# google/compare_gan

Measured on NVIDIA H100. Metric: images/sec G+D step (resnet_cifar10), higher is better.
Workload: dtype tf32

## Files before the change

### compare_gan_b200/csrc/wgmma_tf32.cuh

```cuda
#pragma once
#include <stdint.h>

namespace tc {

template <int N>
__device__ __forceinline__ void wgmma_tf32(float* d, uint64_t da, uint64_t db);

template <>
__device__ __forceinline__ void wgmma_tf32<32>(float* d, uint64_t da, uint64_t db) {
  asm volatile(
      "{\n\t.reg .pred p;\n\tsetp.ne.b32 p, %18, 0;\n\t"
      "wgmma.mma_async.sync.aligned.m64n32k8.f32.tf32.tf32 {%0, %1, %2, %3, %4, %5, %6, %7, %8, %9, %10, %11, %12, %13, %14, %15}, %16, %17, p, 1, 1;\n\t}\n"
      : "+f"(d[0]), "+f"(d[1]), "+f"(d[2]), "+f"(d[3]), "+f"(d[4]), "+f"(d[5]), "+f"(d[6]), "+f"(d[7]), "+f"(d[8]), "+f"(d[9]), "+f"(d[10]), "+f"(d[11]), "+f"(d[12]), "+f"(d[13]), "+f"(d[14]), "+f"(d[15])
      : "l"(da), "l"(db), "r"(1));
}

template <>
__device__ __forceinline__ void wgmma_tf32<64>(float* d, uint64_t da, uint64_t db) {
  asm volatile(
      "{\n\t.reg .pred p;\n\tsetp.ne.b32 p, %34, 0;\n\t"
      "wgmma.mma_async.sync.aligned.m64n64k8.f32.tf32.tf32 {%0, %1, %2, %3, %4, %5, %6, %7, %8, %9, %10, %11, %12, %13, %14, %15, %16, %17, %18, %19, %20, %21, %22, %23, %24, %25, %26, %27, %28, %29, %30, %31}, %32, %33, p, 1, 1;\n\t}\n"
      : "+f"(d[0]), "+f"(d[1]), "+f"(d[2]), "+f"(d[3]), "+f"(d[4]), "+f"(d[5]), "+f"(d[6]), "+f"(d[7]), "+f"(d[8]), "+f"(d[9]), "+f"(d[10]), "+f"(d[11]), "+f"(d[12]), "+f"(d[13]), "+f"(d[14]), "+f"(d[15]), "+f"(d[16]), "+f"(d[17]), "+f"(d[18]), "+f"(d[19]), "+f"(d[20]), "+f"(d[21]), "+f"(d[22]), "+f"(d[23]), "+f"(d[24]), "+f"(d[25]), "+f"(d[26]), "+f"(d[27]), "+f"(d[28]), "+f"(d[29]), "+f"(d[30]), "+f"(d[31])
      : "l"(da), "l"(db), "r"(1));
}

template <>
__device__ __forceinline__ void wgmma_tf32<96>(float* d, uint64_t da, uint64_t db) {
  asm volatile(
      "{\n\t.reg .pred p;\n\tsetp.ne.b32 p, %50, 0;\n\t"
      "wgmma.mma_async.sync.aligned.m64n96k8.f32.tf32.tf32 {%0, %1, %2, %3, %4, %5, %6, %7, %8, %9, %10, %11, %12, %13, %14, %15, %16, %17, %18, %19, %20, %21, %22, %23, %24, %25, %26, %27, %28, %29, %30, %31, %32, %33, %34, %35, %36, %37, %38, %39, %40, %41, %42, %43, %44, %45, %46, %47}, %48, %49, p, 1, 1;\n\t}\n"
      : "+f"(d[0]), "+f"(d[1]), "+f"(d[2]), "+f"(d[3]), "+f"(d[4]), "+f"(d[5]), "+f"(d[6]), "+f"(d[7]), "+f"(d[8]), "+f"(d[9]), "+f"(d[10]), "+f"(d[11]), "+f"(d[12]), "+f"(d[13]), "+f"(d[14]), "+f"(d[15]), "+f"(d[16]), "+f"(d[17]), "+f"(d[18]), "+f"(d[19]), "+f"(d[20]), "+f"(d[21]), "+f"(d[22]), "+f"(d[23]), "+f"(d[24]), "+f"(d[25]), "+f"(d[26]), "+f"(d[27]), "+f"(d[28]), "+f"(d[29]), "+f"(d[30]), "+f"(d[31]), "+f"(d[32]), "+f"(d[33]), "+f"(d[34]), "+f"(d[35]), "+f"(d[36]), "+f"(d[37]), "+f"(d[38]), "+f"(d[39]), "+f"(d[40]), "+f"(d[41]), "+f"(d[42]), "+f"(d[43]), "+f"(d[44]), "+f"(d[45]), "+f"(d[46]), "+f"(d[47])
      : "l"(da), "l"(db), "r"(1));
}

template <>
__device__ __forceinline__ void wgmma_tf32<128>(float* d, uint64_t da, uint64_t db) {
  asm volatile(
      "{\n\t.reg .pred p;\n\tsetp.ne.b32 p, %66, 0;\n\t"
      "wgmma.mma_async.sync.aligned.m64n128k8.f32.tf32.tf32 {%0, %1, %2, %3, %4, %5, %6, %7, %8, %9, %10, %11, %12, %13, %14, %15, %16, %17, %18, %19, %20, %21, %22, %23, %24, %25, %26, %27, %28, %29, %30, %31, %32, %33, %34, %35, %36, %37, %38, %39, %40, %41, %42, %43, %44, %45, %46, %47, %48, %49, %50, %51, %52, %53, %54, %55, %56, %57, %58, %59, %60, %61, %62, %63}, %64, %65, p, 1, 1;\n\t}\n"
      : "+f"(d[0]), "+f"(d[1]), "+f"(d[2]), "+f"(d[3]), "+f"(d[4]), "+f"(d[5]), "+f"(d[6]), "+f"(d[7]), "+f"(d[8]), "+f"(d[9]), "+f"(d[10]), "+f"(d[11]), "+f"(d[12]), "+f"(d[13]), "+f"(d[14]), "+f"(d[15]), "+f"(d[16]), "+f"(d[17]), "+f"(d[18]), "+f"(d[19]), "+f"(d[20]), "+f"(d[21]), "+f"(d[22]), "+f"(d[23]), "+f"(d[24]), "+f"(d[25]), "+f"(d[26]), "+f"(d[27]), "+f"(d[28]), "+f"(d[29]), "+f"(d[30]), "+f"(d[31]), "+f"(d[32]), "+f"(d[33]), "+f"(d[34]), "+f"(d[35]), "+f"(d[36]), "+f"(d[37]), "+f"(d[38]), "+f"(d[39]), "+f"(d[40]), "+f"(d[41]), "+f"(d[42]), "+f"(d[43]), "+f"(d[44]), "+f"(d[45]), "+f"(d[46]), "+f"(d[47]), "+f"(d[48]), "+f"(d[49]), "+f"(d[50]), "+f"(d[51]), "+f"(d[52]), "+f"(d[53]), "+f"(d[54]), "+f"(d[55]), "+f"(d[56]), "+f"(d[57]), "+f"(d[58]), "+f"(d[59]), "+f"(d[60]), "+f"(d[61]), "+f"(d[62]), "+f"(d[63])
      : "l"(da), "l"(db), "r"(1));
}

template <>
__device__ __forceinline__ void wgmma_tf32<160>(float* d, uint64_t da, uint64_t db) {
  asm volatile(
      "{\n\t.reg .pred p;\n\tsetp.ne.b32 p, %82, 0;\n\t"
      "wgmma.mma_async.sync.aligned.m64n160k8.f32.tf32.tf32 {%0, %1, %2, %3, %4, %5, %6, %7, %8, %9, %10, %11, %12, %13, %14, %15, %16, %17, %18, %19, %20, %21, %22, %23, %24, %25, %26, %27, %28, %29, %30, %31, %32, %33, %34, %35, %36, %37, %38, %39, %40, %41, %42, %43, %44, %45, %46, %47, %48, %49, %50, %51, %52, %53, %54, %55, %56, %57, %58, %59, %60, %61, %62, %63, %64, %65, %66, %67, %68, %69, %70, %71, %72, %73, %74, %75, %76, %77, %78, %79}, %80, %81, p, 1, 1;\n\t}\n"
      : "+f"(d[0]), "+f"(d[1]), "+f"(d[2]), "+f"(d[3]), "+f"(d[4]), "+f"(d[5]), "+f"(d[6]), "+f"(d[7]), "+f"(d[8]), "+f"(d[9]), "+f"(d[10]), "+f"(d[11]), "+f"(d[12]), "+f"(d[13]), "+f"(d[14]), "+f"(d[15]), "+f"(d[16]), "+f"(d[17]), "+f"(d[18]), "+f"(d[19]), "+f"(d[20]), "+f"(d[21]), "+f"(d[22]), "+f"(d[23]), "+f"(d[24]), "+f"(d[25]), "+f"(d[26]), "+f"(d[27]), "+f"(d[28]), "+f"(d[29]), "+f"(d[30]), "+f"(d[31]), "+f"(d[32]), "+f"(d[33]), "+f"(d[34]), "+f"(d[35]), "+f"(d[36]), "+f"(d[37]), "+f"(d[38]), "+f"(d[39]), "+f"(d[40]), "+f"(d[41]), "+f"(d[42]), "+f"(d[43]), "+f"(d[44]), "+f"(d[45]), "+f"(d[46]), "+f"(d[47]), "+f"(d[48]), "+f"(d[49]), "+f"(d[50]), "+f"(d[51]), "+f"(d[52]), "+f"(d[53]), "+f"(d[54]), "+f"(d[55]), "+f"(d[56]), "+f"(d[57]), "+f"(d[58]), "+f"(d[59]), "+f"(d[60]), "+f"(d[61]), "+f"(d[62]), "+f"(d[63]), "+f"(d[64]), "+f"(d[65]), "+f"(d[66]), "+f"(d[67]), "+f"(d[68]), "+f"(d[69]), "+f"(d[70]), "+f"(d[71]), "+f"(d[72]), "+f"(d[73]), "+f"(d[74]), "+f"(d[75]), "+f"(d[76]), "+f"(d[77]), "+f"(d[78]), "+f"(d[79])
      : "l"(da), "l"(db), "r"(1));
}

template <>
__device__ __forceinline__ void wgmma_tf32<192>(float* d, uint64_t da, uint64_t db) {
  asm volatile(
      "{\n\t.reg .pred p;\n\tsetp.ne.b32 p, %98, 0;\n\t"
      "wgmma.mma_async.sync.aligned.m64n192k8.f32.tf32.tf32 {%0, %1, %2, %3, %4, %5, %6, %7, %8, %9, %10, %11, %12, %13, %14, %15, %16, %17, %18, %19, %20, %21, %22, %23, %24, %25, %26, %27, %28, %29, %30, %31, %32, %33, %34, %35, %36, %37, %38, %39, %40, %41, %42, %43, %44, %45, %46, %47, %48, %49, %50, %51, %52, %53, %54, %55, %56, %57, %58, %59, %60, %61, %62, %63, %64, %65, %66, %67, %68, %69, %70, %71, %72, %73, %74, %75, %76, %77, %78, %79, %80, %81, %82, %83, %84, %85, %86, %87, %88, %89, %90, %91, %92, %93, %94, %95}, %96, %97, p, 1, 1;\n\t}\n"
      : "+f"(d[0]), "+f"(d[1]), "+f"(d[2]), "+f"(d[3]), "+f"(d[4]), "+f"(d[5]), "+f"(d[6]), "+f"(d[7]), "+f"(d[8]), "+f"(d[9]), "+f"(d[10]), "+f"(d[11]), "+f"(d[12]), "+f"(d[13]), "+f"(d[14]), "+f"(d[15]), "+f"(d[16]), "+f"(d[17]), "+f"(d[18]), "+f"(d[19]), "+f"(d[20]), "+f"(d[21]), "+f"(d[22]), "+f"(d[23]), "+f"(d[24]), "+f"(d[25]), "+f"(d[26]), "+f"(d[27]), "+f"(d[28]), "+f"(d[29]), "+f"(d[30]), "+f"(d[31]), "+f"(d[32]), "+f"(d[33]), "+f"(d[34]), "+f"(d[35]), "+f"(d[36]), "+f"(d[37]), "+f"(d[38]), "+f"(d[39]), "+f"(d[40]), "+f"(d[41]), "+f"(d[42]), "+f"(d[43]), "+f"(d[44]), "+f"(d[45]), "+f"(d[46]), "+f"(d[47]), "+f"(d[48]), "+f"(d[49]), "+f"(d[50]), "+f"(d[51]), "+f"(d[52]), "+f"(d[53]), "+f"(d[54]), "+f"(d[55]), "+f"(d[56]), "+f"(d[57]), "+f"(d[58]), "+f"(d[59]), "+f"(d[60]), "+f"(d[61]), "+f"(d[62]), "+f"(d[63]), "+f"(d[64]), "+f"(d[65]), "+f"(d[66]), "+f"(d[67]), "+f"(d[68]), "+f"(d[69]), "+f"(d[70]), "+f"(d[71]), "+f"(d[72]), "+f"(d[73]), "+f"(d[74]), "+f"(d[75]), "+f"(d[76]), "+f"(d[77]), "+f"(d[78]), "+f"(d[79]), "+f"(d[80]), "+f"(d[81]), "+f"(d[82]), "+f"(d[83]), "+f"(d[84]), "+f"(d[85]), "+f"(d[86]), "+f"(d[87]), "+f"(d[88]), "+f"(d[89]), "+f"(d[90]), "+f"(d[91]), "+f"(d[92]), "+f"(d[93]), "+f"(d[94]), "+f"(d[95])
      : "l"(da), "l"(db), "r"(1));
}

template <>
__device__ __forceinline__ void wgmma_tf32<224>(float* d, uint64_t da, uint64_t db) {
  asm volatile(
      "{\n\t.reg .pred p;\n\tsetp.ne.b32 p, %114, 0;\n\t"
      "wgmma.mma_async.sync.aligned.m64n224k8.f32.tf32.tf32 {%0, %1, %2, %3, %4, %5, %6, %7, %8, %9, %10, %11, %12, %13, %14, %15, %16, %17, %18, %19, %20, %21, %22, %23, %24, %25, %26, %27, %28, %29, %30, %31, %32, %33, %34, %35, %36, %37, %38, %39, %40, %41, %42, %43, %44, %45, %46, %47, %48, %49, %50, %51, %52, %53, %54, %55, %56, %57, %58, %59, %60, %61, %62, %63, %64, %65, %66, %67, %68, %69, %70, %71, %72, %73, %74, %75, %76, %77, %78, %79, %80, %81, %82, %83, %84, %85, %86, %87, %88, %89, %90, %91, %92, %93, %94, %95, %96, %97, %98, %99, %100, %101, %102, %103, %104, %105, %106, %107, %108, %109, %110, %111}, %112, %113, p, 1, 1;\n\t}\n"
      : "+f"(d[0]), "+f"(d[1]), "+f"(d[2]), "+f"(d[3]), "+f"(d[4]), "+f"(d[5]), "+f"(d[6]), "+f"(d[7]), "+f"(d[8]), "+f"(d[9]), "+f"(d[10]), "+f"(d[11]), "+f"(d[12]), "+f"(d[13]), "+f"(d[14]), "+f"(d[15]), "+f"(d[16]), "+f"(d[17]), "+f"(d[18]), "+f"(d[19]), "+f"(d[20]), "+f"(d[21]), "+f"(d[22]), "+f"(d[23]), "+f"(d[24]), "+f"(d[25]), "+f"(d[26]), "+f"(d[27]), "+f"(d[28]), "+f"(d[29]), "+f"(d[30]), "+f"(d[31]), "+f"(d[32]), "+f"(d[33]), "+f"(d[34]), "+f"(d[35]), "+f"(d[36]), "+f"(d[37]), "+f"(d[38]), "+f"(d[39]), "+f"(d[40]), "+f"(d[41]), "+f"(d[42]), "+f"(d[43]), "+f"(d[44]), "+f"(d[45]), "+f"(d[46]), "+f"(d[47]), "+f"(d[48]), "+f"(d[49]), "+f"(d[50]), "+f"(d[51]), "+f"(d[52]), "+f"(d[53]), "+f"(d[54]), "+f"(d[55]), "+f"(d[56]), "+f"(d[57]), "+f"(d[58]), "+f"(d[59]), "+f"(d[60]), "+f"(d[61]), "+f"(d[62]), "+f"(d[63]), "+f"(d[64]), "+f"(d[65]), "+f"(d[66]), "+f"(d[67]), "+f"(d[68]), "+f"(d[69]), "+f"(d[70]), "+f"(d[71]), "+f"(d[72]), "+f"(d[73]), "+f"(d[74]), "+f"(d[75]), "+f"(d[76]), "+f"(d[77]), "+f"(d[78]), "+f"(d[79]), "+f"(d[80]), "+f"(d[81]), "+f"(d[82]), "+f"(d[83]), "+f"(d[84]), "+f"(d[85]), "+f"(d[86]), "+f"(d[87]), "+f"(d[88]), "+f"(d[89]), "+f"(d[90]), "+f"(d[91]), "+f"(d[92]), "+f"(d[93]), "+f"(d[94]), "+f"(d[95]), "+f"(d[96]), "+f"(d[97]), "+f"(d[98]), "+f"(d[99]), "+f"(d[100]), "+f"(d[101]), "+f"(d[102]), "+f"(d[103]), "+f"(d[104]), "+f"(d[105]), "+f"(d[106]), "+f"(d[107]), "+f"(d[108]), "+f"(d[109]), "+f"(d[110]), "+f"(d[111])
      : "l"(da), "l"(db), "r"(1));
}

template <>
__device__ __forceinline__ void wgmma_tf32<256>(float* d, uint64_t da, uint64_t db) {
  asm volatile(
      "{\n\t.reg .pred p;\n\tsetp.ne.b32 p, %130, 0;\n\t"
      "wgmma.mma_async.sync.aligned.m64n256k8.f32.tf32.tf32 {%0, %1, %2, %3, %4, %5, %6, %7, %8, %9, %10, %11, %12, %13, %14, %15, %16, %17, %18, %19, %20, %21, %22, %23, %24, %25, %26, %27, %28, %29, %30, %31, %32, %33, %34, %35, %36, %37, %38, %39, %40, %41, %42, %43, %44, %45, %46, %47, %48, %49, %50, %51, %52, %53, %54, %55, %56, %57, %58, %59, %60, %61, %62, %63, %64, %65, %66, %67, %68, %69, %70, %71, %72, %73, %74, %75, %76, %77, %78, %79, %80, %81, %82, %83, %84, %85, %86, %87, %88, %89, %90, %91, %92, %93, %94, %95, %96, %97, %98, %99, %100, %101, %102, %103, %104, %105, %106, %107, %108, %109, %110, %111, %112, %113, %114, %115, %116, %117, %118, %119, %120, %121, %122, %123, %124, %125, %126, %127}, %128, %129, p, 1, 1;\n\t}\n"
      : "+f"(d[0]), "+f"(d[1]), "+f"(d[2]), "+f"(d[3]), "+f"(d[4]), "+f"(d[5]), "+f"(d[6]), "+f"(d[7]), "+f"(d[8]), "+f"(d[9]), "+f"(d[10]), "+f"(d[11]), "+f"(d[12]), "+f"(d[13]), "+f"(d[14]), "+f"(d[15]), "+f"(d[16]), "+f"(d[17]), "+f"(d[18]), "+f"(d[19]), "+f"(d[20]), "+f"(d[21]), "+f"(d[22]), "+f"(d[23]), "+f"(d[24]), "+f"(d[25]), "+f"(d[26]), "+f"(d[27]), "+f"(d[28]), "+f"(d[29]), "+f"(d[30]), "+f"(d[31]), "+f"(d[32]), "+f"(d[33]), "+f"(d[34]), "+f"(d[35]), "+f"(d[36]), "+f"(d[37]), "+f"(d[38]), "+f"(d[39]), "+f"(d[40]), "+f"(d[41]), "+f"(d[42]), "+f"(d[43]), "+f"(d[44]), "+f"(d[45]), "+f"(d[46]), "+f"(d[47]), "+f"(d[48]), "+f"(d[49]), "+f"(d[50]), "+f"(d[51]), "+f"(d[52]), "+f"(d[53]), "+f"(d[54]), "+f"(d[55]), "+f"(d[56]), "+f"(d[57]), "+f"(d[58]), "+f"(d[59]), "+f"(d[60]), "+f"(d[61]), "+f"(d[62]), "+f"(d[63]), "+f"(d[64]), "+f"(d[65]), "+f"(d[66]), "+f"(d[67]), "+f"(d[68]), "+f"(d[69]), "+f"(d[70]), "+f"(d[71]), "+f"(d[72]), "+f"(d[73]), "+f"(d[74]), "+f"(d[75]), "+f"(d[76]), "+f"(d[77]), "+f"(d[78]), "+f"(d[79]), "+f"(d[80]), "+f"(d[81]), "+f"(d[82]), "+f"(d[83]), "+f"(d[84]), "+f"(d[85]), "+f"(d[86]), "+f"(d[87]), "+f"(d[88]), "+f"(d[89]), "+f"(d[90]), "+f"(d[91]), "+f"(d[92]), "+f"(d[93]), "+f"(d[94]), "+f"(d[95]), "+f"(d[96]), "+f"(d[97]), "+f"(d[98]), "+f"(d[99]), "+f"(d[100]), "+f"(d[101]), "+f"(d[102]), "+f"(d[103]), "+f"(d[104]), "+f"(d[105]), "+f"(d[106]), "+f"(d[107]), "+f"(d[108]), "+f"(d[109]), "+f"(d[110]), "+f"(d[111]), "+f"(d[112]), "+f"(d[113]), "+f"(d[114]), "+f"(d[115]), "+f"(d[116]), "+f"(d[117]), "+f"(d[118]), "+f"(d[119]), "+f"(d[120]), "+f"(d[121]), "+f"(d[122]), "+f"(d[123]), "+f"(d[124]), "+f"(d[125]), "+f"(d[126]), "+f"(d[127])
      : "l"(da), "l"(db), "r"(1));
}

template <int N>
__device__ __forceinline__ void wgmma_tf32_rs(float* d, const uint32_t* a, uint64_t db);

template <>
__device__ __forceinline__ void wgmma_tf32_rs<32>(float* d, const uint32_t* a, uint64_t db) {
  asm volatile(
      "{\n\t.reg .pred p;\n\tsetp.ne.b32 p, %21, 0;\n\t"
      "wgmma.mma_async.sync.aligned.m64n32k8.f32.tf32.tf32 {%0, %1, %2, %3, %4, %5, %6, %7, %8, %9, %10, %11, %12, %13, %14, %15}, {%16, %17, %18, %19}, %20, p, 1, 1;\n\t}\n"
      : "+f"(d[0]), "+f"(d[1]), "+f"(d[2]), "+f"(d[3]), "+f"(d[4]), "+f"(d[5]), "+f"(d[6]), "+f"(d[7]), "+f"(d[8]), "+f"(d[9]), "+f"(d[10]), "+f"(d[11]), "+f"(d[12]), "+f"(d[13]), "+f"(d[14]), "+f"(d[15])
      : "r"(a[0]), "r"(a[1]), "r"(a[2]), "r"(a[3]), "l"(db), "r"(1));
}

template <>
__device__ __forceinline__ void wgmma_tf32_rs<64>(float* d, const uint32_t* a, uint64_t db) {
  asm volatile(
      "{\n\t.reg .pred p;\n\tsetp.ne.b32 p, %37, 0;\n\t"
      "wgmma.mma_async.sync.aligned.m64n64k8.f32.tf32.tf32 {%0, %1, %2, %3, %4, %5, %6, %7, %8, %9, %10, %11, %12, %13, %14, %15, %16, %17, %18, %19, %20, %21, %22, %23, %24, %25, %26, %27, %28, %29, %30, %31}, {%32, %33, %34, %35}, %36, p, 1, 1;\n\t}\n"
      : "+f"(d[0]), "+f"(d[1]), "+f"(d[2]), "+f"(d[3]), "+f"(d[4]), "+f"(d[5]), "+f"(d[6]), "+f"(d[7]), "+f"(d[8]), "+f"(d[9]), "+f"(d[10]), "+f"(d[11]), "+f"(d[12]), "+f"(d[13]), "+f"(d[14]), "+f"(d[15]), "+f"(d[16]), "+f"(d[17]), "+f"(d[18]), "+f"(d[19]), "+f"(d[20]), "+f"(d[21]), "+f"(d[22]), "+f"(d[23]), "+f"(d[24]), "+f"(d[25]), "+f"(d[26]), "+f"(d[27]), "+f"(d[28]), "+f"(d[29]), "+f"(d[30]), "+f"(d[31])
      : "r"(a[0]), "r"(a[1]), "r"(a[2]), "r"(a[3]), "l"(db), "r"(1));
}

template <>
__device__ __forceinline__ void wgmma_tf32_rs<96>(float* d, const uint32_t* a, uint64_t db) {
  asm volatile(
      "{\n\t.reg .pred p;\n\tsetp.ne.b32 p, %53, 0;\n\t"
      "wgmma.mma_async.sync.aligned.m64n96k8.f32.tf32.tf32 {%0, %1, %2, %3, %4, %5, %6, %7, %8, %9, %10, %11, %12, %13, %14, %15, %16, %17, %18, %19, %20, %21, %22, %23, %24, %25, %26, %27, %28, %29, %30, %31, %32, %33, %34, %35, %36, %37, %38, %39, %40, %41, %42, %43, %44, %45, %46, %47}, {%48, %49, %50, %51}, %52, p, 1, 1;\n\t}\n"
      : "+f"(d[0]), "+f"(d[1]), "+f"(d[2]), "+f"(d[3]), "+f"(d[4]), "+f"(d[5]), "+f"(d[6]), "+f"(d[7]), "+f"(d[8]), "+f"(d[9]), "+f"(d[10]), "+f"(d[11]), "+f"(d[12]), "+f"(d[13]), "+f"(d[14]), "+f"(d[15]), "+f"(d[16]), "+f"(d[17]), "+f"(d[18]), "+f"(d[19]), "+f"(d[20]), "+f"(d[21]), "+f"(d[22]), "+f"(d[23]), "+f"(d[24]), "+f"(d[25]), "+f"(d[26]), "+f"(d[27]), "+f"(d[28]), "+f"(d[29]), "+f"(d[30]), "+f"(d[31]), "+f"(d[32]), "+f"(d[33]), "+f"(d[34]), "+f"(d[35]), "+f"(d[36]), "+f"(d[37]), "+f"(d[38]), "+f"(d[39]), "+f"(d[40]), "+f"(d[41]), "+f"(d[42]), "+f"(d[43]), "+f"(d[44]), "+f"(d[45]), "+f"(d[46]), "+f"(d[47])
      : "r"(a[0]), "r"(a[1]), "r"(a[2]), "r"(a[3]), "l"(db), "r"(1));
}

template <>
__device__ __forceinline__ void wgmma_tf32_rs<128>(float* d, const uint32_t* a, uint64_t db) {
  asm volatile(
      "{\n\t.reg .pred p;\n\tsetp.ne.b32 p, %69, 0;\n\t"
      "wgmma.mma_async.sync.aligned.m64n128k8.f32.tf32.tf32 {%0, %1, %2, %3, %4, %5, %6, %7, %8, %9, %10, %11, %12, %13, %14, %15, %16, %17, %18, %19, %20, %21, %22, %23, %24, %25, %26, %27, %28, %29, %30, %31, %32, %33, %34, %35, %36, %37, %38, %39, %40, %41, %42, %43, %44, %45, %46, %47, %48, %49, %50, %51, %52, %53, %54, %55, %56, %57, %58, %59, %60, %61, %62, %63}, {%64, %65, %66, %67}, %68, p, 1, 1;\n\t}\n"
      : "+f"(d[0]), "+f"(d[1]), "+f"(d[2]), "+f"(d[3]), "+f"(d[4]), "+f"(d[5]), "+f"(d[6]), "+f"(d[7]), "+f"(d[8]), "+f"(d[9]), "+f"(d[10]), "+f"(d[11]), "+f"(d[12]), "+f"(d[13]), "+f"(d[14]), "+f"(d[15]), "+f"(d[16]), "+f"(d[17]), "+f"(d[18]), "+f"(d[19]), "+f"(d[20]), "+f"(d[21]), "+f"(d[22]), "+f"(d[23]), "+f"(d[24]), "+f"(d[25]), "+f"(d[26]), "+f"(d[27]), "+f"(d[28]), "+f"(d[29]), "+f"(d[30]), "+f"(d[31]), "+f"(d[32]), "+f"(d[33]), "+f"(d[34]), "+f"(d[35]), "+f"(d[36]), "+f"(d[37]), "+f"(d[38]), "+f"(d[39]), "+f"(d[40]), "+f"(d[41]), "+f"(d[42]), "+f"(d[43]), "+f"(d[44]), "+f"(d[45]), "+f"(d[46]), "+f"(d[47]), "+f"(d[48]), "+f"(d[49]), "+f"(d[50]), "+f"(d[51]), "+f"(d[52]), "+f"(d[53]), "+f"(d[54]), "+f"(d[55]), "+f"(d[56]), "+f"(d[57]), "+f"(d[58]), "+f"(d[59]), "+f"(d[60]), "+f"(d[61]), "+f"(d[62]), "+f"(d[63])
      : "r"(a[0]), "r"(a[1]), "r"(a[2]), "r"(a[3]), "l"(db), "r"(1));
}

}
```

### compare_gan_b200/csrc/wgrad_tc.cu

```cuda
#include "tc_common.cuh"

namespace {

using namespace tc;

constexpr int WG_MAX_STAGES = 4;
constexpr int WG_P = 32;
constexpr int WG_BOX = WG_P * 128;
constexpr int WG_A_BYTES = 4 * WG_BOX;
constexpr int WG_CWARPS = 8;
constexpr int WG_THREADS = 32 * WG_CWARPS + 32;
constexpr int WG_MAX_TAPS = 16;
constexpr int WG_ACC_COLS = 256;

struct WgParams {
  int ntaps;
  int off_h[WG_MAX_TAPS], off_w[WG_MAX_TAPS], amap[WG_MAX_TAPS], bmap[WG_MAX_TAPS], wtap[WG_MAX_TAPS];
  int bw, bh, bni, tiles_w, tiles_h;
  int kblocks, kb_per_split;
  int ci_tiles, co_tiles, bn;
  int cin, cout, taps_total;
  int stages;
  int mt;
  int round_a, round_b;
  float* partial;
  int rows_used;
};

struct BMaps { CUtensorMap m[4]; };

template <int ROWS>
__device__ __forceinline__ void wg_transpose(uint32_t dst, uint32_t src, bool round, int warp, int lane) {
  constexpr int NB = ROWS / 32;
#pragma unroll
  for (int b0 = 0; b0 < NB; b0 += 4) {
    float4 v[4];
#pragma unroll
    for (int b = 0; b < 4; ++b) {
      if (b0 + b >= NB) break;
      const uint32_t s = src + (b0 + b) * WG_BOX + warp * 4 * 128 + lane * 4;
      v[b] = make_float4(lds32(s), lds32(s + 128), lds32(s + 256), lds32(s + 384));
    }
#pragma unroll
    for (int b = 0; b < 4; ++b) {
      if (b0 + b >= NB) break;
      if (round) { v[b].x = rna_tf32(v[b].x); v[b].y = rna_tf32(v[b].y); v[b].z = rna_tf32(v[b].z); v[b].w = rna_tf32(v[b].w); }
      sts128(dst + sw128_offset((b0 + b) * 32 + lane, 4 * warp), v[b]);
    }
  }
}

template <int BN, int MT, bool PART>
__global__ void __launch_bounds__(WG_THREADS, 1)
wgrad_tc_kernel(const __grid_constant__ BMaps tm_x, const __grid_constant__ BMaps tm_dy, const WgParams p) {
  extern __shared__ __align__(1024) uint8_t smem_raw[];
  uint8_t* smem = reinterpret_cast<uint8_t*>((reinterpret_cast<uintptr_t>(smem_raw) + 1023) & ~uintptr_t(1023));
  constexpr int b_bytes = (BN / 32) * WG_BOX;
  constexpr int a_bytes = MT * WG_A_BYTES;
  constexpr int stage_bytes = a_bytes + b_bytes;
  uint8_t* tbuf = smem + p.stages * stage_bytes;
  uint64_t* full_bar = reinterpret_cast<uint64_t*>(tbuf + 2 * stage_bytes);
  uint64_t* empty_bar = full_bar + p.stages;

  const int warp = threadIdx.x >> 5, lane = threadIdx.x & 31;
  int t = blockIdx.x;
  const int co_t = t % p.co_tiles;
  const int u0 = (t / p.co_tiles) * MT;
  const int nu = min(MT, p.ntaps * p.ci_tiles - u0);
  const int tap = u0 / p.ci_tiles;
  const int split = blockIdx.y;
  const int kb0 = split * p.kb_per_split;
  const int kb1 = min(p.kblocks, kb0 + p.kb_per_split);
  const int num_kb = kb1 - kb0;
  const int co0 = co_t * BN;

  if (threadIdx.x == 0) {
    for (int s = 0; s < p.stages; ++s) {
      mbar_init(&full_bar[s], 1);
      mbar_init(&empty_bar[s], WG_CWARPS);
    }
    asm volatile("fence.mbarrier_init.release.cluster;" ::: "memory");
  }
  if (PART) {
    const int tail = (WG_P - p.rows_used) * 128;
    const int words = p.stages * (stage_bytes / WG_BOX) * (tail / 16);
    for (int i = threadIdx.x; i < words; i += WG_THREADS) {
      const int slot = i / (tail / 16), off = i % (tail / 16);
      sts128(smem_u32(smem + slot * WG_BOX + p.rows_used * 128) + off * 16, make_float4(0.f, 0.f, 0.f, 0.f));
    }
  }
  __syncthreads();

  if (warp == WG_CWARPS) {
    if (lane == 0) {
      asm volatile("prefetch.tensormap [%0];" ::"l"(&tm_x.m[p.amap[tap]]) : "memory");
      asm volatile("prefetch.tensormap [%0];" ::"l"(&tm_dy.m[p.bmap[tap]]) : "memory");
      const CUtensorMap* mb = &tm_dy.m[p.bmap[tap]];
      int stage = 0;
      uint32_t phase = 0;
      for (int kb = kb0; kb < kb1; ++kb) {
        int r = kb;
        const int tw = r % p.tiles_w; r /= p.tiles_w;
        const int th = r % p.tiles_h;
        const int tn = r / p.tiles_h;
        const int w0 = tw * p.bw, h0 = th * p.bh, n0 = tn * p.bni;
        mbar_wait(&empty_bar[stage], phase ^ 1);
        uint8_t* sa = smem + stage * stage_bytes;
        uint8_t* sb = sa + a_bytes;
        mbar_expect_tx(&full_bar[stage], PART ? (uint32_t)((nu * 4 + BN / 32) * p.rows_used * 128)
                                              : (uint32_t)(nu * WG_A_BYTES + b_bytes));
        for (int i = 0; i < nu; ++i) {
          const int u = u0 + i, utap = u / p.ci_tiles, ci0 = (u % p.ci_tiles) * 128;
          const CUtensorMap* ma = &tm_x.m[p.amap[utap]];
#pragma unroll
          for (int g = 0; g < 4; ++g)
            tma_load_4d(sa + i * WG_A_BYTES + g * WG_BOX, ma, &full_bar[stage], ci0 + g * 32, w0 + p.off_w[utap],
                        h0 + p.off_h[utap], n0);
        }
        for (int g = 0; g < BN / 32; ++g) tma_load_4d(sb + g * WG_BOX, mb, &full_bar[stage], co0 + g * 32, w0, h0, n0);
        if (++stage == p.stages) { stage = 0; phase ^= 1; }
      }
    }
    return;
  }

  const int wg = warp >> 2;
  float acc[MT][BN / 2];
#pragma unroll
  for (int u = 0; u < MT; ++u)
#pragma unroll
    for (int i = 0; i < BN / 2; ++i) acc[u][i] = 0.f;
  int stage = 0;
  uint32_t phase = 0;
  for (int kb = 0; kb < num_kb; ++kb) {
    mbar_wait(&full_bar[stage], phase);
    const uint32_t s_addr = smem_u32(smem + stage * stage_bytes);
    const uint32_t t_addr = smem_u32(tbuf + (kb & 1) * stage_bytes);
    for (int i = 0; i < nu; ++i) wg_transpose<128>(t_addr + i * WG_A_BYTES, s_addr + i * WG_A_BYTES, p.round_a, warp, lane);
    wg_transpose<BN>(t_addr + a_bytes, s_addr + a_bytes, p.round_b, warp, lane);
    __syncwarp();
    if (lane == 0) mbar_arrive(&empty_bar[stage]);
    fence_proxy_async();
    wgmma_wait<0>();
    named_bar(1, 32 * WG_CWARPS);
#pragma unroll
    for (int u = 0; u < MT; ++u)
#pragma unroll
      for (int i = 0; i < BN / 2; ++i) acc_fence(acc[u][i]);
    wgmma_fence();
#pragma unroll
    for (int u = 0; u < MT; ++u) {
#pragma unroll
      for (int k = 0; k < WG_P / 8; ++k)
        wgmma_tf32<BN>(acc[u], make_desc(t_addr + u * WG_A_BYTES + wg * (WG_A_BYTES / 2) + k * 32),
                       make_desc(t_addr + a_bytes + k * 32));
    }
    wgmma_commit();
    if (++stage == p.stages) { stage = 0; phase ^= 1; }
  }
  wgmma_wait<0>();
#pragma unroll
  for (int u = 0; u < MT; ++u)
#pragma unroll
    for (int i = 0; i < BN / 2; ++i) acc_fence(acc[u][i]);
  const int c2 = (lane & 3) * 2;
  const bool vec2 = (p.cout & 1) == 0;
#pragma unroll
  for (int u = 0; u < MT; ++u) {
    if (u >= nu) continue;
    const int uu = u0 + u, utap = uu / p.ci_tiles, ci0 = (uu % p.ci_tiles) * 128;
#pragma unroll
    for (int h = 0; h < 2; ++h) {
      const int row = wg * 64 + (warp & 3) * 16 + (lane >> 2) + h * 8;
      if (ci0 + row >= p.cin) continue;
      float* orow = p.partial + (((long long)split * p.taps_total + p.wtap[utap]) * p.cin + ci0 + row) * p.cout + co0;
#pragma unroll
      for (int j = 0; j < BN / 8; ++j) {
        const int c = j * 8 + c2;
        if (co0 + c >= p.cout) continue;
        if (vec2) {
          *reinterpret_cast<float2*>(orow + c) = make_float2(acc[u][4 * j + 2 * h], acc[u][4 * j + 2 * h + 1]);
        } else {
          orow[c] = acc[u][4 * j + 2 * h];
          if (co0 + c + 1 < p.cout) orow[c + 1] = acc[u][4 * j + 2 * h + 1];
        }
      }
    }
  }
}

bool box32(int n, int h, int w, int* bw, int* bh, int* bni) {
  if (n < 1 || h < 1 || w < 1) return false;
  int b = w < 32 ? w : 32;
  if (32 % b != 0 || w % b != 0) return false;
  int hh = 32 / b; if (hh > h) hh = h;
  if (h % hh != 0) return false;
  int ni = 32 / (b * hh);
  if (ni < 1 || b * hh * ni != 32 || n % ni != 0) return false;
  *bw = b; *bh = hh; *bni = ni;
  return true;
}

bool box_any(int n, int h, int w, int* bw, int* bh, int* bni) {
  if (n < 1 || h < 1 || w < 1 || 32 % w == 0 || w % 32 == 0) return false;
  long long best = -1;
  for (int b = w < 32 ? w : 32; b >= 1; --b)
    for (int hh = 32 / b < h ? 32 / b : h; hh >= 1; --hh) {
      const int ni = 32 / (b * hh) < n ? 32 / (b * hh) : n;
      const long long kb = (long long)((w + b - 1) / b) * ((h + hh - 1) / hh) * ((n + ni - 1) / ni);
      if (best < 0 || kb < best) { best = kb; *bw = b; *bh = hh; *bni = ni; }
    }
  return true;
}

bool wg_box(int n, int h, int w, bool per_image, int* bw, int* bh, int* bni) {
  return box32(n, h, w, bw, bh, bni) || (!per_image && box_any(n, h, w, bw, bh, bni));
}

int pick_bn(int ncols) {
  if (ncols <= 256 && ncols % 4 == 0) return (ncols + 31) / 32 * 32;
  if (ncols % 32) return 0;
  if (ncols <= 256) return ncols;
  if (ncols % 256 == 0) return 256;
  if (ncols % 192 == 0) return 192;
  if (ncols % 128 == 0) return 128;
  return 0;
}

size_t wg_smem(size_t stage_bytes, size_t budget, int* stages) {
  long long s = (long long)(budget / stage_bytes) - 2;
  if (s > WG_MAX_STAGES) s = WG_MAX_STAGES;
  if (s < 2) s = 2;
  *stages = (int)s;
  return (size_t)(s + 2) * stage_bytes + 1024 + 256;
}

template <int BN, int MT, bool PART>
int wg_launch_t(cgan_ctx* ctx, dim3 grid, size_t smem, const BMaps& tm_x, const BMaps& tm_dy, const WgParams& p) {
  static bool attr_set = false;
  if (!attr_set) {
    CGAN_CUDA(ctx, cudaFuncSetAttribute(wgrad_tc_kernel<BN, MT, PART>, cudaFuncAttributeMaxDynamicSharedMemorySize,
                                        227 * 1024));
    attr_set = true;
  }
  wgrad_tc_kernel<BN, MT, PART><<<grid, WG_THREADS, smem, ctx->stream>>>(tm_x, tm_dy, p);
  CGAN_LAUNCHED(ctx);
  return CGAN_OK;
}

int wg_launch(cgan_ctx* ctx, dim3 grid, size_t smem, const BMaps& tm_x, const BMaps& tm_dy, const WgParams& p) {
#define WG_CASE(BN, MT)                                                                                        \
  if (p.bn == BN && p.mt == MT)                                                                                \
    return p.rows_used < WG_P ? wg_launch_t<BN, MT, true>(ctx, grid, smem, tm_x, tm_dy, p)                    \
                              : wg_launch_t<BN, MT, false>(ctx, grid, smem, tm_x, tm_dy, p);
  WG_CASE(32, 1) WG_CASE(64, 1) WG_CASE(96, 1) WG_CASE(128, 1) WG_CASE(160, 1) WG_CASE(192, 1) WG_CASE(224, 1)
  WG_CASE(256, 1) WG_CASE(32, 2) WG_CASE(64, 2) WG_CASE(96, 2) WG_CASE(128, 2)
#undef WG_CASE
  return cgan_fail(ctx, CGAN_ERR_UNSUPPORTED, "%s: no kernel for this column tile%s", "cgan_wgrad_tc");
}

}

bool cgan_wgrad_tc_fits(const TcWgrad& g) {
  int bw, bh, bni;
  return wg_box(g.dy.n, g.dy.h, g.dy.w, g.per_image, &bw, &bh, &bni) && (!g.per_image || (bni == 1 && g.dy.n <= 65535)) &&
         g.x.ch > 0 && g.x.ch % 32 == 0 &&
         pick_bn(g.dy.ch) != 0 && g.taps.ntaps >= 1 && g.taps.ntaps <= WG_MAX_TAPS && al16(g.x.in) && al16(g.dy.in) &&
         al16(g.dw);
}

int cgan_wgrad_tc(cgan_ctx* ctx, const TcWgrad& g) {
  if (!cgan_wgrad_tc_fits(g)) return cgan_fail(ctx, CGAN_ERR_UNSUPPORTED, "%s: shape%s", "cgan_wgrad_tc");
  WgParams p;
  memset(&p, 0, sizeof(p));
  const int n = g.dy.n, gh = g.dy.h, gw = g.dy.w;
  p.round_a = g.x.tf32 ? 0 : 1;
  p.round_b = g.dy.tf32 ? 0 : 1;
  wg_box(n, gh, gw, g.per_image, &p.bw, &p.bh, &p.bni);
  p.rows_used = p.bw * p.bh * p.bni;
  p.tiles_w = (gw + p.bw - 1) / p.bw;
  p.tiles_h = (gh + p.bh - 1) / p.bh;
  p.kblocks = (int)((long long)p.tiles_w * p.tiles_h * ((n + p.bni - 1) / p.bni));
  p.bn = pick_bn(g.dy.ch);
  p.ci_tiles = (g.x.ch + 127) / 128;
  p.co_tiles = (g.dy.ch + p.bn - 1) / p.bn;
  p.cin = g.x.ch; p.cout = g.dy.ch; p.taps_total = g.taps_total;
  const ConvTaps& t = g.taps;
  p.ntaps = t.ntaps;
  for (int i = 0; i < t.ntaps; ++i) {
    p.off_h[i] = t.off_h[i]; p.off_w[i] = t.off_w[i]; p.wtap[i] = t.wtap[i];
    p.amap[i] = g.taps_view_dy ? 0 : t.view[i];
    p.bmap[i] = g.taps_view_dy ? t.view[i] : 0;
  }
  const int units = p.ci_tiles * t.ntaps;
  bool same_b = true;
  for (int i = 1; i < t.ntaps; ++i) same_b = same_b && p.bmap[i] == p.bmap[0];
  p.mt = (!g.per_image && ctx->tc_mt_max >= 2 && same_b && units >= 2 && 2 * p.bn <= WG_ACC_COLS) ? 2 : 1;
  const size_t stage_bytes = (size_t)p.mt * WG_A_BYTES + (size_t)(p.bn / 32) * WG_BOX;
  const long long tiles = (long long)p.co_tiles * ((units + p.mt - 1) / p.mt);
  int splits;
  size_t smem;
  if (g.per_image) {
    p.kb_per_split = gh * gw / WG_P;
    splits = n;
    smem = wg_smem(stage_bytes, 110 * 1024, &p.stages);
  } else {
    const bool two_ctas = wg_smem(stage_bytes, 110 * 1024, &p.stages) <= 113 * 1024;
    splits = (int)((2ll * ctx->num_sms) / tiles);
    int max_splits = p.kblocks / 8 > 0 ? p.kblocks / 8 : 1;
    if (splits > max_splits) splits = max_splits;
    if (splits < 1) splits = 1;
    p.kb_per_split = (p.kblocks + splits - 1) / splits;
    splits = (p.kblocks + p.kb_per_split - 1) / p.kb_per_split;
    smem = wg_smem(stage_bytes, two_ctas ? 110 * 1024 : 220 * 1024, &p.stages);
  }

  const bool reduce = !g.per_image && splits > 1;
  const long long wn = (long long)p.taps_total * p.cin * p.cout;
  p.partial = g.dw;
  if (reduce) {
    void* ws = nullptr;
    int rc = cgan_ws(ctx, (size_t)splits * wn * sizeof(float), &ws);
    if (rc) return rc;
    p.partial = reinterpret_cast<float*>(ws);
  }

  BMaps tm_x, tm_dy;
  memset(&tm_x, 0, sizeof(tm_x));
  memset(&tm_dy, 0, sizeof(tm_dy));
  for (int v = 0; v < 4; ++v)
    if (!make_view_map(&tm_x.m[v], g.x, v, p.bw, p.bh, p.bni, CU_TENSOR_MAP_SWIZZLE_NONE) ||
        !make_view_map(&tm_dy.m[v], g.dy, v, p.bw, p.bh, p.bni, CU_TENSOR_MAP_SWIZZLE_NONE))
      return cgan_fail(ctx, CGAN_ERR_CUDA, "%s: cuTensorMapEncodeTiled failed%s", "cgan_wgrad_tc");
  int rc = wg_launch(ctx, dim3((unsigned)tiles, (unsigned)splits), smem, tm_x, tm_dy, p);
  if (rc || !reduce) return rc;
  return cgan_splitk_reduce(ctx, g.dw, p.partial, wn, splits);
}
```

Measured before the change: 23010.

## Feed wgrad WGMMA A operand from registers and double-buffer transposed B

The weight-gradient kernel no longer transposes the activation (A) tile through shared memory. It loads A fragments straight into registers from a 128B-swizzled TMA layout and issues register-sourced wgmma instructions at the wider N sizes added to the header. Only the B tile is still transposed, into a double buffer guarded by new buf_free barriers, so the next block's transpose can overlap in-flight MMAs. The shared-memory budget changes to match, and when MT*BN>=256 the block gets extra producer warps plus setmaxnreg register reallocation. The risks are register pressure from the large accumulators plus fragments, and correctness of the intricate fragment and channel mapping.

Measured after the change: 23850, median of 6. 3.6% higher.

```diff
diff --git a/compare_gan_b200/csrc/wgmma_tf32.cuh b/compare_gan_b200/csrc/wgmma_tf32.cuh
--- a/compare_gan_b200/csrc/wgmma_tf32.cuh
+++ b/compare_gan_b200/csrc/wgmma_tf32.cuh
@@ -117,4 +117,40 @@
       : "r"(a[0]), "r"(a[1]), "r"(a[2]), "r"(a[3]), "l"(db), "r"(1));
 }
 
+template <>
+__device__ __forceinline__ void wgmma_tf32_rs<160>(float* d, const uint32_t* a, uint64_t db) {
+  asm volatile(
+      "{\n\t.reg .pred p;\n\tsetp.ne.b32 p, %85, 0;\n\t"
+      "wgmma.mma_async.sync.aligned.m64n160k8.f32.tf32.tf32 {%0, %1, %2, %3, %4, %5, %6, %7, %8, %9, %10, %11, %12, %13, %14, %15, %16, %17, %18, %19, %20, %21, %22, %23, %24, %25, %26, %27, %28, %29, %30, %31, %32, %33, %34, %35, %36, %37, %38, %39, %40, %41, %42, %43, %44, %45, %46, %47, %48, %49, %50, %51, %52, %53, %54, %55, %56, %57, %58, %59, %60, %61, %62, %63, %64, %65, %66, %67, %68, %69, %70, %71, %72, %73, %74, %75, %76, %77, %78, %79}, {%80, %81, %82, %83}, %84, p, 1, 1;\n\t}\n"
+      : "+f"(d[0]), "+f"(d[1]), "+f"(d[2]), "+f"(d[3]), "+f"(d[4]), "+f"(d[5]), "+f"(d[6]), "+f"(d[7]), "+f"(d[8]), "+f"(d[9]), "+f"(d[10]), "+f"(d[11]), "+f"(d[12]), "+f"(d[13]), "+f"(d[14]), "+f"(d[15]), "+f"(d[16]), "+f"(d[17]), "+f"(d[18]), "+f"(d[19]), "+f"(d[20]), "+f"(d[21]), "+f"(d[22]), "+f"(d[23]), "+f"(d[24]), "+f"(d[25]), "+f"(d[26]), "+f"(d[27]), "+f"(d[28]), "+f"(d[29]), "+f"(d[30]), "+f"(d[31]), "+f"(d[32]), "+f"(d[33]), "+f"(d[34]), "+f"(d[35]), "+f"(d[36]), "+f"(d[37]), "+f"(d[38]), "+f"(d[39]), "+f"(d[40]), "+f"(d[41]), "+f"(d[42]), "+f"(d[43]), "+f"(d[44]), "+f"(d[45]), "+f"(d[46]), "+f"(d[47]), "+f"(d[48]), "+f"(d[49]), "+f"(d[50]), "+f"(d[51]), "+f"(d[52]), "+f"(d[53]), "+f"(d[54]), "+f"(d[55]), "+f"(d[56]), "+f"(d[57]), "+f"(d[58]), "+f"(d[59]), "+f"(d[60]), "+f"(d[61]), "+f"(d[62]), "+f"(d[63]), "+f"(d[64]), "+f"(d[65]), "+f"(d[66]), "+f"(d[67]), "+f"(d[68]), "+f"(d[69]), "+f"(d[70]), "+f"(d[71]), "+f"(d[72]), "+f"(d[73]), "+f"(d[74]), "+f"(d[75]), "+f"(d[76]), "+f"(d[77]), "+f"(d[78]), "+f"(d[79])
+      : "r"(a[0]), "r"(a[1]), "r"(a[2]), "r"(a[3]), "l"(db), "r"(1));
 }
+
+template <>
+__device__ __forceinline__ void wgmma_tf32_rs<192>(float* d, const uint32_t* a, uint64_t db) {
+  asm volatile(
+      "{\n\t.reg .pred p;\n\tsetp.ne.b32 p, %101, 0;\n\t"
+      "wgmma.mma_async.sync.aligned.m64n192k8.f32.tf32.tf32 {%0, %1, %2, %3, %4, %5, %6, %7, %8, %9, %10, %11, %12, %13, %14, %15, %16, %17, %18, %19, %20, %21, %22, %23, %24, %25, %26, %27, %28, %29, %30, %31, %32, %33, %34, %35, %36, %37, %38, %39, %40, %41, %42, %43, %44, %45, %46, %47, %48, %49, %50, %51, %52, %53, %54, %55, %56, %57, %58, %59, %60, %61, %62, %63, %64, %65, %66, %67, %68, %69, %70, %71, %72, %73, %74, %75, %76, %77, %78, %79, %80, %81, %82, %83, %84, %85, %86, %87, %88, %89, %90, %91, %92, %93, %94, %95}, {%96, %97, %98, %99}, %100, p, 1, 1;\n\t}\n"
+      : "+f"(d[0]), "+f"(d[1]), "+f"(d[2]), "+f"(d[3]), "+f"(d[4]), "+f"(d[5]), "+f"(d[6]), "+f"(d[7]), "+f"(d[8]), "+f"(d[9]), "+f"(d[10]), "+f"(d[11]), "+f"(d[12]), "+f"(d[13]), "+f"(d[14]), "+f"(d[15]), "+f"(d[16]), "+f"(d[17]), "+f"(d[18]), "+f"(d[19]), "+f"(d[20]), "+f"(d[21]), "+f"(d[22]), "+f"(d[23]), "+f"(d[24]), "+f"(d[25]), "+f"(d[26]), "+f"(d[27]), "+f"(d[28]), "+f"(d[29]), "+f"(d[30]), "+f"(d[31]), "+f"(d[32]), "+f"(d[33]), "+f"(d[34]), "+f"(d[35]), "+f"(d[36]), "+f"(d[37]), "+f"(d[38]), "+f"(d[39]), "+f"(d[40]), "+f"(d[41]), "+f"(d[42]), "+f"(d[43]), "+f"(d[44]), "+f"(d[45]), "+f"(d[46]), "+f"(d[47]), "+f"(d[48]), "+f"(d[49]), "+f"(d[50]), "+f"(d[51]), "+f"(d[52]), "+f"(d[53]), "+f"(d[54]), "+f"(d[55]), "+f"(d[56]), "+f"(d[57]), "+f"(d[58]), "+f"(d[59]), "+f"(d[60]), "+f"(d[61]), "+f"(d[62]), "+f"(d[63]), "+f"(d[64]), "+f"(d[65]), "+f"(d[66]), "+f"(d[67]), "+f"(d[68]), "+f"(d[69]), "+f"(d[70]), "+f"(d[71]), "+f"(d[72]), "+f"(d[73]), "+f"(d[74]), "+f"(d[75]), "+f"(d[76]), "+f"(d[77]), "+f"(d[78]), "+f"(d[79]), "+f"(d[80]), "+f"(d[81]), "+f"(d[82]), "+f"(d[83]), "+f"(d[84]), "+f"(d[85]), "+f"(d[86]), "+f"(d[87]), "+f"(d[88]), "+f"(d[89]), "+f"(d[90]), "+f"(d[91]), "+f"(d[92]), "+f"(d[93]), "+f"(d[94]), "+f"(d[95])
+      : "r"(a[0]), "r"(a[1]), "r"(a[2]), "r"(a[3]), "l"(db), "r"(1));
+}
+
+template <>
+__device__ __forceinline__ void wgmma_tf32_rs<224>(float* d, const uint32_t* a, uint64_t db) {
+  asm volatile(
+      "{\n\t.reg .pred p;\n\tsetp.ne.b32 p, %117, 0;\n\t"
+      "wgmma.mma_async.sync.aligned.m64n224k8.f32.tf32.tf32 {%0, %1, %2, %3, %4, %5, %6, %7, %8, %9, %10, %11, %12, %13, %14, %15, %16, %17, %18, %19, %20, %21, %22, %23, %24, %25, %26, %27, %28, %29, %30, %31, %32, %33, %34, %35, %36, %37, %38, %39, %40, %41, %42, %43, %44, %45, %46, %47, %48, %49, %50, %51, %52, %53, %54, %55, %56, %57, %58, %59, %60, %61, %62, %63, %64, %65, %66, %67, %68, %69, %70, %71, %72, %73, %74, %75, %76, %77, %78, %79, %80, %81, %82, %83, %84, %85, %86, %87, %88, %89, %90, %91, %92, %93, %94, %95, %96, %97, %98, %99, %100, %101, %102, %103, %104, %105, %106, %107, %108, %109, %110, %111}, {%112, %113, %114, %115}, %116, p, 1, 1;\n\t}\n"
+      : "+f"(d[0]), "+f"(d[1]), "+f"(d[2]), "+f"(d[3]), "+f"(d[4]), "+f"(d[5]), "+f"(d[6]), "+f"(d[7]), "+f"(d[8]), "+f"(d[9]), "+f"(d[10]), "+f"(d[11]), "+f"(d[12]), "+f"(d[13]), "+f"(d[14]), "+f"(d[15]), "+f"(d[16]), "+f"(d[17]), "+f"(d[18]), "+f"(d[19]), "+f"(d[20]), "+f"(d[21]), "+f"(d[22]), "+f"(d[23]), "+f"(d[24]), "+f"(d[25]), "+f"(d[26]), "+f"(d[27]), "+f"(d[28]), "+f"(d[29]), "+f"(d[30]), "+f"(d[31]), "+f"(d[32]), "+f"(d[33]), "+f"(d[34]), "+f"(d[35]), "+f"(d[36]), "+f"(d[37]), "+f"(d[38]), "+f"(d[39]), "+f"(d[40]), "+f"(d[41]), "+f"(d[42]), "+f"(d[43]), "+f"(d[44]), "+f"(d[45]), "+f"(d[46]), "+f"(d[47]), "+f"(d[48]), "+f"(d[49]), "+f"(d[50]), "+f"(d[51]), "+f"(d[52]), "+f"(d[53]), "+f"(d[54]), "+f"(d[55]), "+f"(d[56]), "+f"(d[57]), "+f"(d[58]), "+f"(d[59]), "+f"(d[60]), "+f"(d[61]), "+f"(d[62]), "+f"(d[63]), "+f"(d[64]), "+f"(d[65]), "+f"(d[66]), "+f"(d[67]), "+f"(d[68]), "+f"(d[69]), "+f"(d[70]), "+f"(d[71]), "+f"(d[72]), "+f"(d[73]), "+f"(d[74]), "+f"(d[75]), "+f"(d[76]), "+f"(d[77]), "+f"(d[78]), "+f"(d[79]), "+f"(d[80]), "+f"(d[81]), "+f"(d[82]), "+f"(d[83]), "+f"(d[84]), "+f"(d[85]), "+f"(d[86]), "+f"(d[87]), "+f"(d[88]), "+f"(d[89]), "+f"(d[90]), "+f"(d[91]), "+f"(d[92]), "+f"(d[93]), "+f"(d[94]), "+f"(d[95]), "+f"(d[96]), "+f"(d[97]), "+f"(d[98]), "+f"(d[99]), "+f"(d[100]), "+f"(d[101]), "+f"(d[102]), "+f"(d[103]), "+f"(d[104]), "+f"(d[105]), "+f"(d[106]), "+f"(d[107]), "+f"(d[108]), "+f"(d[109]), "+f"(d[110]), "+f"(d[111])
+      : "r"(a[0]), "r"(a[1]), "r"(a[2]), "r"(a[3]), "l"(db), "r"(1));
+}
+
+template <>
+__device__ __forceinline__ void wgmma_tf32_rs<256>(float* d, const uint32_t* a, uint64_t db) {
+  asm volatile(
+      "{\n\t.reg .pred p;\n\tsetp.ne.b32 p, %133, 0;\n\t"
+      "wgmma.mma_async.sync.aligned.m64n256k8.f32.tf32.tf32 {%0, %1, %2, %3, %4, %5, %6, %7, %8, %9, %10, %11, %12, %13, %14, %15, %16, %17, %18, %19, %20, %21, %22, %23, %24, %25, %26, %27, %28, %29, %30, %31, %32, %33, %34, %35, %36, %37, %38, %39, %40, %41, %42, %43, %44, %45, %46, %47, %48, %49, %50, %51, %52, %53, %54, %55, %56, %57, %58, %59, %60, %61, %62, %63, %64, %65, %66, %67, %68, %69, %70, %71, %72, %73, %74, %75, %76, %77, %78, %79, %80, %81, %82, %83, %84, %85, %86, %87, %88, %89, %90, %91, %92, %93, %94, %95, %96, %97, %98, %99, %100, %101, %102, %103, %104, %105, %106, %107, %108, %109, %110, %111, %112, %113, %114, %115, %116, %117, %118, %119, %120, %121, %122, %123, %124, %125, %126, %127}, {%128, %129, %130, %131}, %132, p, 1, 1;\n\t}\n"
+      : "+f"(d[0]), "+f"(d[1]), "+f"(d[2]), "+f"(d[3]), "+f"(d[4]), "+f"(d[5]), "+f"(d[6]), "+f"(d[7]), "+f"(d[8]), "+f"(d[9]), "+f"(d[10]), "+f"(d[11]), "+f"(d[12]), "+f"(d[13]), "+f"(d[14]), "+f"(d[15]), "+f"(d[16]), "+f"(d[17]), "+f"(d[18]), "+f"(d[19]), "+f"(d[20]), "+f"(d[21]), "+f"(d[22]), "+f"(d[23]), "+f"(d[24]), "+f"(d[25]), "+f"(d[26]), "+f"(d[27]), "+f"(d[28]), "+f"(d[29]), "+f"(d[30]), "+f"(d[31]), "+f"(d[32]), "+f"(d[33]), "+f"(d[34]), "+f"(d[35]), "+f"(d[36]), "+f"(d[37]), "+f"(d[38]), "+f"(d[39]), "+f"(d[40]), "+f"(d[41]), "+f"(d[42]), "+f"(d[43]), "+f"(d[44]), "+f"(d[45]), "+f"(d[46]), "+f"(d[47]), "+f"(d[48]), "+f"(d[49]), "+f"(d[50]), "+f"(d[51]), "+f"(d[52]), "+f"(d[53]), "+f"(d[54]), "+f"(d[55]), "+f"(d[56]), "+f"(d[57]), "+f"(d[58]), "+f"(d[59]), "+f"(d[60]), "+f"(d[61]), "+f"(d[62]), "+f"(d[63]), "+f"(d[64]), "+f"(d[65]), "+f"(d[66]), "+f"(d[67]), "+f"(d[68]), "+f"(d[69]), "+f"(d[70]), "+f"(d[71]), "+f"(d[72]), "+f"(d[73]), "+f"(d[74]), "+f"(d[75]), "+f"(d[76]), "+f"(d[77]), "+f"(d[78]), "+f"(d[79]), "+f"(d[80]), "+f"(d[81]), "+f"(d[82]), "+f"(d[83]), "+f"(d[84]), "+f"(d[85]), "+f"(d[86]), "+f"(d[87]), "+f"(d[88]), "+f"(d[89]), "+f"(d[90]), "+f"(d[91]), "+f"(d[92]), "+f"(d[93]), "+f"(d[94]), "+f"(d[95]), "+f"(d[96]), "+f"(d[97]), "+f"(d[98]), "+f"(d[99]), "+f"(d[100]), "+f"(d[101]), "+f"(d[102]), "+f"(d[103]), "+f"(d[104]), "+f"(d[105]), "+f"(d[106]), "+f"(d[107]), "+f"(d[108]), "+f"(d[109]), "+f"(d[110]), "+f"(d[111]), "+f"(d[112]), "+f"(d[113]), "+f"(d[114]), "+f"(d[115]), "+f"(d[116]), "+f"(d[117]), "+f"(d[118]), "+f"(d[119]), "+f"(d[120]), "+f"(d[121]), "+f"(d[122]), "+f"(d[123]), "+f"(d[124]), "+f"(d[125]), "+f"(d[126]), "+f"(d[127])
+      : "r"(a[0]), "r"(a[1]), "r"(a[2]), "r"(a[3]), "l"(db), "r"(1));
+}
+
+}
diff --git a/compare_gan_b200/csrc/wgrad_tc.cu b/compare_gan_b200/csrc/wgrad_tc.cu
--- a/compare_gan_b200/csrc/wgrad_tc.cu
+++ b/compare_gan_b200/csrc/wgrad_tc.cu
@@ -9,7 +9,7 @@
 constexpr int WG_BOX = WG_P * 128;
 constexpr int WG_A_BYTES = 4 * WG_BOX;
 constexpr int WG_CWARPS = 8;
-constexpr int WG_THREADS = 32 * WG_CWARPS + 32;
+constexpr int WG_THREADS = 32 * WG_CWARPS + 128;
 constexpr int WG_MAX_TAPS = 16;
 constexpr int WG_ACC_COLS = 256;
 
@@ -50,6 +50,25 @@
   }
 }
 
+__device__ __forceinline__ void frag_fence(uint32_t& r) { asm volatile("" : "+r"(r)::"memory"); }
+
+__device__ __forceinline__ int wg_a_channel(int warp, int lane) {
+  const int r = lane >> 2;
+  return 4 * (2 * (warp & 1) + (r >> 2) + 4 * ((r >> 1) & 1)) + 2 * (r & 1);
+}
+
+template <int GK>
+__device__ __forceinline__ void wg_load_a(uint32_t (&f)[GK][4], uint32_t src, uint32_t lo, uint32_t hi, bool round) {
+#pragma unroll
+  for (int e = 0; e < GK; ++e) {
+    float2 a = lds64(src + e * 1024 + lo), b = lds64(src + e * 1024 + hi);
+    if (round) { a.x = rna_tf32(a.x); a.y = rna_tf32(a.y); b.x = rna_tf32(b.x); b.y = rna_tf32(b.y); }
+    f[e][0] = __float_as_uint(a.x); f[e][1] = __float_as_uint(a.y); f[e][2] = __float_as_uint(b.x); f[e][3] = __float_as_uint(b.y);
+#pragma unroll
+    for (int i = 0; i < 4; ++i) frag_fence(f[e][i]);
+  }
+}
+
 template <int BN, int MT, bool PART>
 __global__ void __launch_bounds__(WG_THREADS, 1)
 wgrad_tc_kernel(const __grid_constant__ BMaps tm_x, const __grid_constant__ BMaps tm_dy, const WgParams p) {
@@ -59,8 +78,9 @@
   constexpr int a_bytes = MT * WG_A_BYTES;
   constexpr int stage_bytes = a_bytes + b_bytes;
   uint8_t* tbuf = smem + p.stages * stage_bytes;
-  uint64_t* full_bar = reinterpret_cast<uint64_t*>(tbuf + 2 * stage_bytes);
+  uint64_t* full_bar = reinterpret_cast<uint64_t*>(tbuf + 2 * b_bytes);
   uint64_t* empty_bar = full_bar + p.stages;
+  uint64_t* buf_free = empty_bar + p.stages;
 
   const int warp = threadIdx.x >> 5, lane = threadIdx.x & 31;
   int t = blockIdx.x;
@@ -79,6 +99,7 @@
       mbar_init(&full_bar[s], 1);
       mbar_init(&empty_bar[s], WG_CWARPS);
     }
+    for (int b = 0; b < 2; ++b) mbar_init(&buf_free[b], WG_CWARPS);
     asm volatile("fence.mbarrier_init.release.cluster;" ::: "memory");
   }
   if (PART) {
@@ -91,8 +112,10 @@
   }
   __syncthreads();
 
-  if (warp == WG_CWARPS) {
-    if (lane == 0) {
+  constexpr bool REALLOC = MT * BN >= 256;
+  if (warp >= WG_CWARPS) {
+    if (REALLOC) asm volatile("setmaxnreg.dec.sync.aligned.u32 40;" ::: "memory");
+    if (warp == WG_CWARPS && lane == 0) {
       asm volatile("prefetch.tensormap [%0];" ::"l"(&tm_x.m[p.amap[tap]]) : "memory");
       asm volatile("prefetch.tensormap [%0];" ::"l"(&tm_dy.m[p.bmap[tap]]) : "memory");
       const CUtensorMap* mb = &tm_dy.m[p.bmap[tap]];
@@ -124,36 +147,52 @@
     return;
   }
 
+  if (REALLOC) asm volatile("setmaxnreg.inc.sync.aligned.u32 232;" ::: "memory");
+  constexpr int GK = 2 * MT;
   const int wg = warp >> 2;
+  const int cib = wg_a_channel(warp, lane), q = lane & 3;
+  const uint32_t a_box = (2 * wg + ((warp >> 1) & 1)) * WG_BOX + (cib & 3) * 4;
+  const uint32_t a_lo = a_box + q * 128 + ((((cib >> 2) ^ q) & 7) << 4);
+  const uint32_t a_hi = a_box + (q + 4) * 128 + ((((cib >> 2) ^ (q + 4)) & 7) << 4);
+  const bool all_units = MT == 1 || nu == MT;
   float acc[MT][BN / 2];
 #pragma unroll
   for (int u = 0; u < MT; ++u)
 #pragma unroll
     for (int i = 0; i < BN / 2; ++i) acc[u][i] = 0.f;
+  uint32_t fa[2][GK][4];
   int stage = 0;
   uint32_t phase = 0;
   for (int kb = 0; kb < num_kb; ++kb) {
+    const int h = kb & 1;
     mbar_wait(&full_bar[stage], phase);
     const uint32_t s_addr = smem_u32(smem + stage * stage_bytes);
-    const uint32_t t_addr = smem_u32(tbuf + (kb & 1) * stage_bytes);
-    for (int i = 0; i < nu; ++i) wg_transpose<128>(t_addr + i * WG_A_BYTES, s_addr + i * WG_A_BYTES, p.round_a, warp, lane);
-    wg_transpose<BN>(t_addr + a_bytes, s_addr + a_bytes, p.round_b, warp, lane);
+    const uint32_t t_addr = smem_u32(tbuf + h * b_bytes);
+    wgmma_wait<1>();
+    wg_load_a<GK>(fa[0], s_addr, a_lo, a_hi, p.round_a);
+    if (kb >= 2) mbar_wait(&buf_free[h], ((kb >> 1) & 1) ^ 1);
+    wg_transpose<BN>(t_addr, s_addr + a_bytes, p.round_b, warp, lane);
+    fence_proxy_async();
+    named_bar(1, 32 * WG_CWARPS);
+#pragma unroll
+    for (int u = 0; u < MT; ++u)
+#pragma unroll
+      for (int i = 0; i < BN / 2; ++i) acc_fence(acc[u][i]);
+    wgmma_fence();
+#pragma unroll
+    for (int e = 0; e < GK; ++e)
+      wgmma_tf32_rs<BN>(acc[e / 4], fa[0][e], make_desc(t_addr + (e % 4) * 32));
+    wgmma_commit();
+    wgmma_wait<1>();
+    if (kb >= 1 && lane == 0) mbar_arrive(&buf_free[h ^ 1]);
+    if (all_units) wg_load_a<GK>(fa[1], s_addr + (GK / 4) * WG_A_BYTES + (GK % 4) * 1024, a_lo, a_hi, p.round_a);
     __syncwarp();
     if (lane == 0) mbar_arrive(&empty_bar[stage]);
-    fence_proxy_async();
-    wgmma_wait<0>();
-    named_bar(1, 32 * WG_CWARPS);
-#pragma unroll
-    for (int u = 0; u < MT; ++u)
-#pragma unroll
-      for (int i = 0; i < BN / 2; ++i) acc_fence(acc[u][i]);
     wgmma_fence();
-#pragma unroll
-    for (int u = 0; u < MT; ++u) {
-#pragma unroll
-      for (int k = 0; k < WG_P / 8; ++k)
-        wgmma_tf32<BN>(acc[u], make_desc(t_addr + u * WG_A_BYTES + wg * (WG_A_BYTES / 2) + k * 32),
-                       make_desc(t_addr + a_bytes + k * 32));
+    if (all_units) {
+#pragma unroll
+      for (int e = 0; e < GK; ++e)
+        wgmma_tf32_rs<BN>(acc[(GK + e) / 4], fa[1][e], make_desc(t_addr + ((GK + e) % 4) * 32));
     }
     wgmma_commit();
     if (++stage == p.stages) { stage = 0; phase ^= 1; }
@@ -171,7 +210,7 @@
     const int uu = u0 + u, utap = uu / p.ci_tiles, ci0 = (uu % p.ci_tiles) * 128;
 #pragma unroll
     for (int h = 0; h < 2; ++h) {
-      const int row = wg * 64 + (warp & 3) * 16 + (lane >> 2) + h * 8;
+      const int row = (2 * wg + ((warp >> 1) & 1)) * 32 + cib + h;
       if (ci0 + row >= p.cin) continue;
       float* orow = p.partial + (((long long)split * p.taps_total + p.wtap[utap]) * p.cin + ci0 + row) * p.cout + co0;
 #pragma unroll
@@ -227,12 +266,12 @@
   return 0;
 }
 
-size_t wg_smem(size_t stage_bytes, size_t budget, int* stages) {
-  long long s = (long long)(budget / stage_bytes) - 2;
+size_t wg_smem(size_t stage_bytes, size_t t_bytes, size_t budget, int* stages) {
+  long long s = ((long long)budget - 2 * (long long)t_bytes) / (long long)stage_bytes;
   if (s > WG_MAX_STAGES) s = WG_MAX_STAGES;
   if (s < 2) s = 2;
   *stages = (int)s;
-  return (size_t)(s + 2) * stage_bytes + 1024 + 256;
+  return (size_t)s * stage_bytes + 2 * t_bytes + 1024 + 256;
 }
 
 template <int BN, int MT, bool PART>
@@ -296,23 +335,24 @@
   bool same_b = true;
   for (int i = 1; i < t.ntaps; ++i) same_b = same_b && p.bmap[i] == p.bmap[0];
   p.mt = (!g.per_image && ctx->tc_mt_max >= 2 && same_b && units >= 2 && 2 * p.bn <= WG_ACC_COLS) ? 2 : 1;
-  const size_t stage_bytes = (size_t)p.mt * WG_A_BYTES + (size_t)(p.bn / 32) * WG_BOX;
+  const size_t t_bytes = (size_t)(p.bn / 32) * WG_BOX;
+  const size_t stage_bytes = (size_t)p.mt * WG_A_BYTES + t_bytes;
   const long long tiles = (long long)p.co_tiles * ((units + p.mt - 1) / p.mt);
   int splits;
   size_t smem;
   if (g.per_image) {
     p.kb_per_split = gh * gw / WG_P;
     splits = n;
-    smem = wg_smem(stage_bytes, 110 * 1024, &p.stages);
+    smem = wg_smem(stage_bytes, t_bytes, 110 * 1024, &p.stages);
   } else {
-    const bool two_ctas = wg_smem(stage_bytes, 110 * 1024, &p.stages) <= 113 * 1024;
+    const bool two_ctas = stage_bytes <= 24 * 1024;
     splits = (int)((2ll * ctx->num_sms) / tiles);
     int max_splits = p.kblocks / 8 > 0 ? p.kblocks / 8 : 1;
     if (splits > max_splits) splits = max_splits;
     if (splits < 1) splits = 1;
     p.kb_per_split = (p.kblocks + splits - 1) / splits;
     splits = (p.kblocks + p.kb_per_split - 1) / p.kb_per_split;
-    smem = wg_smem(stage_bytes, two_ctas ? 110 * 1024 : 220 * 1024, &p.stages);
+    smem = wg_smem(stage_bytes, t_bytes, two_ctas ? 110 * 1024 : 225 * 1024, &p.stages);
   }
 
   const bool reduce = !g.per_image && splits > 1;
@@ -329,7 +369,7 @@
   memset(&tm_x, 0, sizeof(tm_x));
   memset(&tm_dy, 0, sizeof(tm_dy));
   for (int v = 0; v < 4; ++v)
-    if (!make_view_map(&tm_x.m[v], g.x, v, p.bw, p.bh, p.bni, CU_TENSOR_MAP_SWIZZLE_NONE) ||
+    if (!make_view_map(&tm_x.m[v], g.x, v, p.bw, p.bh, p.bni, CU_TENSOR_MAP_SWIZZLE_128B) ||
         !make_view_map(&tm_dy.m[v], g.dy, v, p.bw, p.bh, p.bni, CU_TENSOR_MAP_SWIZZLE_NONE))
       return cgan_fail(ctx, CGAN_ERR_CUDA, "%s: cuTensorMapEncodeTiled failed%s", "cgan_wgrad_tc");
   int rc = wg_launch(ctx, dim3((unsigned)tiles, (unsigned)splits), smem, tm_x, tm_dy, p);
```
